# ntnu-arl/mimosa

Measured on AMD Instinct MI355X. Metric: ICP corr+residual Mpts/sec, 131k-pt scan vs 5M-pt map, 1/2/4/8 GPU, higher is better.
Workload: dtype f64; 1 GPU; configs[1]: OS0-128 131072-pt scan vs 4963194-pt local map (511380 voxels, 2x5 rooms), k=5 point-to-plane, ENWIDE params, cold linearize per step; parallelism=single GPU, exact_fallback_queries=0

## Files before the change

### mimosa_amd/csrc/icp_kernels.hip

```cpp
#include <hip/hip_runtime.h>

#include <cstdlib>

#include "icp_device.hpp"

#ifndef MH_PRUNE_TRIPS
#define MH_PRUNE_TRIPS (trip == 1 || trip == 2)
#endif
#ifndef MH_PIPE
#define MH_PIPE 4
#endif
#ifndef MH_XCD_PIECES
#define MH_XCD_PIECES 2
#endif
#ifndef MH_PIPE_SMALL
#define MH_PIPE_SMALL 4
#endif
#include "map_device.hpp"
#include "math3.hpp"
#include "wave_dpp.hpp"

namespace mh
{
namespace
// ... 93 lines not shown
#endif
#ifdef MH_TIMELINE
#define MH_STAMP4(ptr, i)                                                                                          \
  do {                                                                                                             \
    if ((ptr) && (threadIdx.x & 63) == 0 && (threadIdx.x >> 6) < static_cast<unsigned int>(NW))                    \
      (ptr)[(static_cast<size_t>(block_id) * NW + (threadIdx.x >> 6)) * 16 + (i)] = __builtin_amdgcn_s_memtime();  \
  } while (0)
#else
#define MH_STAMP4(ptr, i) do { } while (0)
#endif
#define MH_STAMP_C2(ptr, i) MH_STAMP(ptr, i)

struct KeyConsts
{
  uint32_t ymask, ymagic, kmask, xmask, xmagic;
};

__device__ __forceinline__ void cmp_exch(uint32_t & a, uint32_t & b)
{
  const uint32_t lo = min(a, b);
  b = max(a, b);
  a = lo;
}

typedef float f32x2 __attribute__((ext_vector_type(2)));
__device__ __forceinline__ uint32_t med3_u32(uint32_t a, uint32_t b, uint32_t c)
{
  uint32_t r;
  asm("v_med3_u32 %0, %1, %2, %3" : "=v"(r) : "v"(a), "v"(b), "v"(c));
  return r;
}
__device__ __forceinline__ f32x2 coarse_dist2(const KeyConsts & kc, uint32_t wa, uint32_t wb, float ofx, float mfy, float ofz)
{
  const f32x2 xm = {__uint_as_float((wa & kc.xmask) | kc.xmagic), __uint_as_float((wb & kc.xmask) | kc.xmagic)};
  const f32x2 x = xm - 8388608.0f;
  const f32x2 y = {__uint_as_float((wa & kc.ymask) | kc.ymagic), __uint_as_float((wb & kc.ymask) | kc.ymagic)};
  const f32x2 z = {static_cast<float>(wa >> 20), static_cast<float>(wb >> 20)};
  const f32x2 dx = x + ofx, dy = y - mfy, dz = z + ofz;
  f32x2 d = dy * dy;
  d = __builtin_elementwise_fma(dx, dx, d);
  d = __builtin_elementwise_fma(dz, dz, d);
  return d;
}
template <int KK>
__device__ __forceinline__ void merge_quad(uint32_t (&ck)[KK], const KeyConsts & kc, const uint4 qw, float ofx, float mfy, float ofz,
                                           uint32_t pb, uint32_t vcnt)
{
  const f32x2 da = coarse_dist2(kc, qw.x, qw.y, ofx, mfy, ofz), db = coarse_dist2(kc, qw.z, qw.w, ofx, mfy, ofz);
  uint32_t k0 = (__float_as_uint(da.x) & kc.kmask) | pb;
  uint32_t k1 = (__float_as_uint(da.y) & kc.kmask) | (pb | 1u);
  uint32_t k2 = (__float_as_uint(db.x) & kc.kmask) | (pb | 2u);
  uint32_t k3 = (__float_as_uint(db.y) & kc.kmask) | (pb | 3u);
  k0 = vcnt > 0u ? k0 : 0xFFFFFFFFu;
  k1 = vcnt > 1u ? k1 : 0xFFFFFFFFu;
  k2 = vcnt > 2u ? k2 : 0xFFFFFFFFu;
  k3 = vcnt > 3u ? k3 : 0xFFFFFFFFu;
  if constexpr (KK == 8) {
    cmp_exch(k0, k1); cmp_exch(k2, k3); cmp_exch(k0, k2); cmp_exch(k1, k3); cmp_exch(k1, k2);
    const uint32_t q[4] = {k3, k2, k1, k0};
#pragma unroll
    for (int i = 0; i < 4; ++i) {
      const uint32_t hi = med3_u32(ck[i], ck[4 + i], q[i]);
      ck[i] = min(ck[i], q[i]);
      ck[4 + i] = hi;
    }
    cmp_exch(ck[0], ck[2]); cmp_exch(ck[1], ck[3]); cmp_exch(ck[4], ck[6]); cmp_exch(ck[5], ck[7]);
    cmp_exch(ck[0], ck[1]); cmp_exch(ck[2], ck[3]); cmp_exch(ck[4], ck[5]); cmp_exch(ck[6], ck[7]);
  } else {
    const uint32_t kq[4] = {k0, k1, k2, k3};
#pragma unroll
    for (int c = 0; c < 4; ++c) {
      uint32_t t = kq[c];
#pragma unroll
      for (int i = 0; i < KK - 1; ++i) {
        const uint32_t lo = min(ck[i], t);
        t = max(ck[i], t);
        ck[i] = lo;
      }
      ck[KK - 1] = min(ck[KK - 1], t);
    }
  }
}

struct ScanStage
{
  uint4 quad;
  float4 ofs;
  uint32_t pb;
  uint32_t vcnt;
};
template <int NOFF>
struct ScanCursor
{
  uint32_t rem;
  int o_cur = 0;
  uint32_t qd = 8u, nq_cur = 0u;
  uint64_t qc0, qc1;

  __device__ __forceinline__ ScanStage advance(const uint32_t * list, int lds_stride, const float4 * lut4, const uint4 * qbuckets)
  {
    const bool sw = (qd >= nq_cur) && rem != 0u;
    o_cur = sw ? __builtin_ctz(rem) : o_cur;
    rem = sw ? (rem & (rem - 1u)) : rem;
    qd = sw ? 0u : qd;
    if constexpr (NOFF <= 21)
      nq_cur = static_cast<uint32_t>(qc0 >> (3 * o_cur)) & 7u;
    else
      nq_cur = static_cast<uint32_t>((o_cur < 21 ? qc0 : qc1) >> (3 * (o_cur < 21 ? o_cur : o_cur - 21))) & 7u;
    const uint32_t e = list[o_cur * lds_stride];
    ScanStage st;
    st.ofs = lut4[o_cur];
    uint32_t qidx = (e >> 5) * (kBucketStride / 4) + min(qd, static_cast<uint32_t>(kBucketStride / 4 - 1));
    st.quad = qbuckets[qidx];
    const uint32_t q4 = qd << 2;
    st.vcnt = static_cast<uint32_t>(min(max(static_cast<int>(e & 31u) - static_cast<int>(q4), 0), 4));
    st.pb = (static_cast<uint32_t>(o_cur) << 5) | q4;
    ++qd;
    return st;
  }
};

template <int K, int KK, int NOFF>
__device__ __forceinline__ uint32_t prune_keep_mask(const uint32_t (&ck)[KK], const float (&boxd)[NOFF], int k, float err_g,
                                                    uint32_t kth_given = 0xFFFFFFFFu)
{
  uint32_t kth = kth_given;
#pragma unroll
  for (int i = 0; i < K; ++i)
    if (i == k - 1) kth = min(kth, ck[i]);
  const float kv = __uint_as_float(kth & ~0x3FFu) * (1.0f + 2.5e-4f);
  const float r_up = sqrtf(kv) * (1.0f + 2e-6f) + err_g;
  const float b_up = kth != 0xFFFFFFFFu ? r_up * r_up : 3.0e38f;
  uint32_t keep = ~0u;
#pragma unroll
  for (int b = 1; b < NOFF; ++b) keep &= boxd[b] > b_up ? ~(1u << b) : ~0u;
  return keep;
}

template <int NOFF>
__device__ __forceinline__ void box_dists(const float qg0, const float qg1, const float qg2, float (&boxd)[NOFF])
{
  constexpr int row = NOFF == 7 ? 1 : (NOFF == 19 ? 2 : 3);
  constexpr float kQ = static_cast<float>(1 << kQuantBits);
  const float marg = 1e-2f;
  const float gxm = fmaxf(qg0 - marg, 0.f), gxp = fmaxf(kQ - qg0 - marg, 0.f);
  const float gym = fmaxf(qg1 - marg, 0.f), gyp = fmaxf(kQ - qg1 - marg, 0.f);
  const float gzm = fmaxf(qg2 - marg, 0.f), gzp = fmaxf(kQ - qg2 - marg, 0.f);
  const float g2x[3] = {gxm * gxm, 0.f, gxp * gxp}, g2y[3] = {gym * gym, 0.f, gyp * gyp}, g2z[3] = {gzm * gzm, 0.f, gzp * gzp};
#pragma unroll
  for (int b = 0; b < NOFF; ++b) {
    const uint32_t ent = kScan.ent[row][b];
    boxd[b] = g2x[ent & 3u] + g2y[(ent >> 2) & 3u] + g2z[(ent >> 4) & 3u];
  }
}

template <int KK, int NOFF, int PIPE>
__device__ __forceinline__ uint32_t scan_trip(ScanCursor<NOFF> & cur, ScanStage (&stage)[PIPE], uint32_t (&ck)[KK], const KeyConsts & kc,
                                              const uint32_t * list, int lds_stride, const float4 * lut4, const uint4 * qbuckets,
                                              const float cx0, const float cy1, const float cz2, uint32_t & n_scanned)
{
  uint32_t live_quads = 0u;
#pragma unroll
  for (int u = 0; u < PIPE; ++u) {
    const ScanStage st = stage[u];
    stage[u] = cur.advance(list, lds_stride, lut4, qbuckets);
    n_scanned += st.vcnt;
    live_quads += st.vcnt ? 1u : 0u;
    merge_quad<KK>(ck, kc, st.quad, st.ofs.x + cx0, cy1 - st.ofs.y, st.ofs.z + cz2, st.pb, st.vcnt);
  }
  return live_quads;
}

template <int CTRL>
__device__ __forceinline__ uint32_t quad_pull(uint32_t v)
{
  return static_cast<uint32_t>(__builtin_amdgcn_update_dpp(0, static_cast<int>(v), CTRL, 0xF, 0xF, false));
}
template <int CTRL>
__device__ __forceinline__ void quad_merge8(uint32_t (&ck)[8])
{
  uint32_t o[8];
#pragma unroll
  for (int i = 0; i < 8; ++i) o[i] = quad_pull<CTRL>(ck[7 - i]);
#pragma unroll
  for (int i = 0; i < 8; ++i) ck[i] = min(ck[i], o[i]);
  cmp_exch(ck[0], ck[4]); cmp_exch(ck[1], ck[5]); cmp_exch(ck[2], ck[6]); cmp_exch(ck[3], ck[7]);
  cmp_exch(ck[0], ck[2]); cmp_exch(ck[1], ck[3]); cmp_exch(ck[4], ck[6]); cmp_exch(ck[5], ck[7]);
  cmp_exch(ck[0], ck[1]); cmp_exch(ck[2], ck[3]); cmp_exch(ck[4], ck[5]); cmp_exch(ck[6], ck[7]);
}
template <int QL>
__device__ __forceinline__ void group_merge8(uint32_t (&ck)[8])
{
  if constexpr (QL >= 2) quad_merge8<0xB1>(ck);
  if constexpr (QL >= 4) quad_merge8<0x4E>(ck);
}
template <int QL>
__device__ __forceinline__ uint32_t group_min(uint32_t v)
{
  if constexpr (QL >= 2) v = min(v, quad_pull<0xB1>(v));
  if constexpr (QL >= 4) v = min(v, quad_pull<0x4E>(v));
  return v;
}
template <int QL>
__device__ __forceinline__ uint32_t group_or(uint32_t v)
{
  if constexpr (QL >= 2) v |= quad_pull<0xB1>(v);
  if constexpr (QL >= 4) v |= quad_pull<0x4E>(v);
  return v;
}
__device__ __forceinline__ uint32_t prefix_parity(uint32_t x)
{
  uint32_t y = x;
  y ^= y << 1;
  y ^= y << 2;
  y ^= y << 4;
  y ^= y << 8;
  y ^= y << 16;
  return y;
}
template <int QL>
__device__ __forceinline__ uint32_t deal_bits(uint32_t x, uint32_t sub)
{
  if constexpr (QL == 1) return x;
  const uint32_t odd = x & prefix_parity(x);
  uint32_t m = (sub & 1u) ? (x & ~odd) : odd;
  if constexpr (QL == 4) {
    const uint32_t odd2 = m & prefix_parity(m);
    m = (sub & 2u) ? (m & ~odd2) : odd2;
  }
  return m;
}

template <int KK>
struct KnnPoints
{
  float4 pt[KK];
  uint32_t member;
};
constexpr int knn_survivors(int K) { return K + 3 + (K > 5 ? 1 : 0); }
template <int K, int NOFF, bool FAST = false, int PIPE = MH_PIPE, int QL = 1>
__device__ __forceinline__ uint32_t knn_query(const MapView & map, const double q0, const double q1, const double q2,
                                              int k, uint32_t * list, int lds_stride, const uint32_t * scan_lut,
                                              uint32_t (&bi)[K], double & dk, bool & fell_back, uint32_t & n_scanned,
                                              unsigned long long * dbg = nullptr, KnnPoints<knn_survivors(K)> * fast = nullptr)
{
  (void)dbg;
  (void)fast;
  static_assert(QL == 1 || (FAST && knn_survivors(K) == 8), "several lanes per query: the k = 5 fast path's top-8 only");
  [[maybe_unused]] const uint32_t sub = QL > 1 ? (threadIdx.x & static_cast<uint32_t>(QL - 1)) : 0u;
  fell_back = false;
  constexpr int KK = knn_survivors(K);
  constexpr int row = NOFF == 7 ? 1 : (NOFF == 19 ? 2 : 3);
  const double u0 = q0 * map.inv_leaf, u1 = q1 * map.inv_leaf, u2 = q2 * map.inv_leaf;
  const int cx = fast_floor(u0), cy = fast_floor(u1), cz = fast_floor(u2);
  constexpr int m = kBlockDim - 1;
  const int bx = cx >> kBlockLog2, by = cy >> kBlockLog2, bz = cz >> kBlockLog2;
  int blk_id;
  {
    const uint64_t key = pack_coord_key(bx, by, bz);
    const int klo = static_cast<int>(static_cast<uint32_t>(key)), khi = static_cast<int>(static_cast<uint32_t>(key >> 32));
    uint32_t h = block_hash(bx, by, bz) & map.mask;
    int4 e = map.table[h];
    while (e.y != -1 && !(e.x == klo && e.y == khi)) {
      h = (h + 1) & map.mask;
      e = map.table[h];
    }
    constexpr int kB = 1 << (kVoxCoordBits - 1 - kBlockLog2);
    const bool in_range = ((static_cast<uint32_t>(bx + kB) | static_cast<uint32_t>(by + kB) | static_cast<uint32_t>(bz + kB)) >> (kVoxCoordBits - kBlockLog2)) == 0u;
    blk_id = (e.y != -1 && in_range) ? e.z : -1;
  }
  MH_STAMP(dbg, 8);
  uint32_t col[9][3];
  {
    const uint32_t * tab = map.cells + static_cast<size_t>(blk_id < 0 ? 0 : blk_id) * kCellsPerBlock +
                           halo_index(cx & m, cy & m, cz & m);
#pragma unroll
    for (int c = 0; c < 9; ++c) {
      const uint32_t * p = tab + ((c / 3 - 1) * kHaloDim + (c % 3 - 1)) * kHaloDim - 1;
      col[c][0] = p[0];
      col[c][1] = p[1];
      col[c][2] = p[2];
    }
  }
  uint32_t cell[NOFF];
#pragma unroll
  for (int b = 0; b < NOFF; ++b) {
    const uint32_t ent = kScan.ent[row][b];
    const int ox = static_cast<int>(ent & 3u), oy = static_cast<int>((ent >> 2) & 3u), oz = static_cast<int>((ent >> 4) & 3u);
    cell[b] = (blk_id >= 0 && static_cast<int>(ent >> 6) < map.n_off) ? col[ox * 3 + oy][oz] : kEmptyCell;
  }
#ifdef MH_TIMELINE
  asm volatile("s_waitcnt vmcnt(0)" ::: "memory");
#endif
  MH_STAMP(dbg, 9);
  uint32_t amask = 0u, total_ref = 0u;
  uint64_t qc0 = 0, qc1 = 0;
#pragma unroll
  for (int o = 0; o < NOFF; ++o) {
    static_assert(kEmptyCell == 0u, "an empty cell reads as (voxel 0, count 0): a mapped index and no candidates, without a select");
    list[o * lds_stride] = cell[o];
    const uint32_t c = cell[o] & 31u;
    amask |= (c ? 1u : 0u) << o;
    total_ref += c;
    const uint64_t nq = (c + 3u) >> 2;
    if (o < 21)
      qc0 |= nq << (3 * o);
    else
      qc1 |= nq << (3 * (o - 21));
  }
  MH_STAMP(dbg, 1);

  constexpr float kErrG = 0.9f;
  constexpr double kQ_d = static_cast<double>(1 << kQuantBits);
  const float qg0 = static_cast<float>((u0 - static_cast<double>(cx)) * kQ_d);
  const float qg1 = static_cast<float>((u1 - static_cast<double>(cy)) * kQ_d);
  const float qg2 = static_cast<float>((u2 - static_cast<double>(cz)) * kQ_d);
  uint32_t ck[KK];
#pragma unroll
  for (int i = 0; i < KK; ++i) ck[i] = 0xFFFFFFFFu;
  KeyConsts kc{0xFFC00u, 0x46000000u, ~0x3FFu, 0x3FFu, 0x4B000000u};
  asm volatile("" : "+v"(kc.ymask), "+v"(kc.ymagic), "+v"(kc.kmask), "+v"(kc.xmask), "+v"(kc.xmagic));

  n_scanned = 0;
  if constexpr (QL == 1) {
    if (amask & 1u) {
      const uint32_t cc = cell[0] & 31u;
      const uint4 * b = map.qbuckets + static_cast<size_t>(cell[0] >> 5) * (kBucketStride / 4);
      n_scanned += cc;
      const float ofx = 0.5f - qg0, ofy = 0.5f - qg1, ofz = 0.5f - qg2;
      uint4 qw[kBucketStride / 4];
#pragma unroll
      for (int u = 0; u < kBucketStride / 4; ++u) qw[u] = b[static_cast<uint32_t>(4 * u) < cc ? u : 0];
#pragma unroll
      for (int u = 0; u < kBucketStride / 4; ++u) {
        if (static_cast<uint32_t>(4 * u) < cc) merge_quad<KK>(ck, kc, qw[u], ofx, 8192.0f - ofy, ofz, static_cast<uint32_t>(4 * u), min(cc - static_cast<uint32_t>(4 * u), 4u));
      }
    }
  } else {
    const uint32_t cc = cell[0] & 31u;
    const uint4 * b = map.qbuckets + static_cast<size_t>(cell[0] >> 5) * (kBucketStride / 4);
    const float ofx = 0.5f - qg0, ofy = 0.5f - qg1, ofz = 0.5f - qg2;
    constexpr int NJ = (kBucketStride / 4 + QL - 1) / QL;
    uint4 qw[NJ];
#pragma unroll
    for (int j = 0; j < NJ; ++j) qw[j] = b[min(static_cast<uint32_t>(j * QL) + sub, static_cast<uint32_t>(kBucketStride / 4 - 1))];
#pragma unroll
    for (int j = 0; j < NJ; ++j) {
      const uint32_t u4 = 4u * (static_cast<uint32_t>(j * QL) + sub);
      const uint32_t vc = static_cast<uint32_t>(min(max(static_cast<int>(cc) - static_cast<int>(u4), 0), 4));
      n_scanned += vc;
      merge_quad<KK>(ck, kc, qw[j], ofx, 8192.0f - ofy, ofz, min(u4, 28u), vc);
    }
    group_merge8<QL>(ck);
  }
  MH_STAMP(dbg, 10);
  float boxd[NOFF];
  box_dists<NOFF>(qg0, qg1, qg2, boxd);
  uint32_t rem = amask & ~1u;
  rem &= prune_keep_mask<K, KK, NOFF>(ck, boxd, k, kErrG);
  [[maybe_unused]] uint32_t kth_group = 0xFFFFFFFFu;
  if constexpr (QL > 1) {
#pragma unroll
    for (int i = 0; i < K; ++i)
      if (i == k - 1) kth_group = ck[i];
    rem = deal_bits<QL>(rem, sub);
    if (sub != 0u) {
#pragma unroll
      for (int i = 0; i < KK; ++i) ck[i] = 0xFFFFFFFFu;
    }
  }
  uint32_t alive = rem;

  MH_STAMP(dbg, 11);
  {
    constexpr int kPipe = PIPE;
    const float4 * lut4 = reinterpret_cast<const float4 *>(scan_lut);
    const float cx0 = 0.5f - qg0, cy1 = 8192.0f - 0.5f + qg1, cz2 = 0.5f - qg2;
    ScanCursor<NOFF> cur;
    cur.rem = rem;
    cur.qc0 = qc0;
    cur.qc1 = qc1;
    ScanStage stage[kPipe];
#pragma unroll
    for (int u = 0; u < kPipe; ++u) stage[u] = cur.advance(list, lds_stride, lut4, map.qbuckets);
    for (int trip = 0;; ++trip) {
      if (!__any(static_cast<int>(stage[0].vcnt))) break;
      if (MH_PRUNE_TRIPS) {
        if constexpr (QL > 1) {
          uint32_t mine = kth_group;
#pragma unroll
          for (int i = 0; i < K; ++i)
            if (i == k - 1) mine = min(mine, ck[i]);
          kth_group = group_min<QL>(mine);
        }
        const uint32_t keep = prune_keep_mask<K, KK, NOFF>(ck, boxd, k, kErrG, kth_group);
        cur.rem &= keep;
        alive &= keep;
      }
      scan_trip<KK, NOFF, kPipe>(cur, stage, ck, kc, list, lds_stride, lut4, map.qbuckets, cx0, cy1, cz2, n_scanned);
    }
    rem = cur.rem;
  }
  if constexpr (QL > 1) {
    group_merge8<QL>(ck);
    alive = group_or<QL>(alive & ~rem);
    rem = 0u;
  }
  const uint32_t lane = threadIdx.x & 63u;
  const uint64_t act = __ballot(1);
  const uint32_t nact = static_cast<uint32_t>(__popcll(act));
  const uint32_t rank = static_cast<uint32_t>(__popcll(act & ((1ull << lane) - 1ull)));
  const uint32_t scanned_mask = (amask & 1u) | (alive & ~rem);
  MH_STAMP(dbg, 2);

  double bd[K];
  uint32_t br[K];
#pragma unroll
  for (int i = 0; i < K; ++i) {
    bd[i] = kDblMax;
    bi[i] = 0xFFFFFFFFu;
    br[i] = 0xFFFFFFFFu;
  }
  {
    uint32_t sidx[KK], srank[KK];
    float4 sc[KK];
#pragma unroll
    for (int u = 0; u < KK; ++u) {
      const uint32_t p = ck[u] & 0x3FFu;
      const int b = min(static_cast<int>(p >> 5), NOFF - 1);
      const uint32_t e = list[b * lds_stride];
      sidx[u] = (e >> 5) * kBucketStride + (p & 31u);
      sc[u] = map.buckets[sidx[u]];
      srank[u] = (scan_lut[4 * b + 3] << 5) | (p & 31u);
    }
    if constexpr (FAST) {
      unsigned long long d[KK];
      uint32_t rk[KK];
#pragma unroll
      for (int u = 0; u < KK; ++u) {
        const double du = sq_dist3(static_cast<double>(sc[u].x) - q0, static_cast<double>(sc[u].y) - q1, static_cast<double>(sc[u].z) - q2);
        d[u] = static_cast<unsigned long long>(__double_as_longlong(ck[u] != 0xFFFFFFFFu ? du : kDblMax));
        rk[u] = 0u;
      }
#pragma unroll
      for (int u = 0; u < KK; ++u)
#pragma unroll
        for (int v = u + 1; v < KK; ++v) {
          const bool lt = d[u] < d[v];
          rk[v] += lt ? 1u : 0u;
          rk[u] += lt ? 0u : 1u;
        }
      unsigned long long dk_bits = static_cast<unsigned long long>(__double_as_longlong(kDblMax)), dn_bits = ~0ull;
#pragma unroll
      for (int u = 0; u < KK; ++u) {
        dk_bits = rk[u] == static_cast<uint32_t>(k - 1) ? d[u] : dk_bits;
        dn_bits = rk[u] == static_cast<uint32_t>(k) ? d[u] : dn_bits;
      }
      uint32_t member = 0u;
#pragma unroll
      for (int u = 0; u < KK; ++u) {
        const bool valid = ck[u] != 0xFFFFFFFFu;
        member |= (valid && rk[u] < static_cast<uint32_t>(k)) ? (1u << u) : 0u;
        fast->pt[u] = sc[u];
      }
      if (__any(static_cast<int>(dk_bits == dn_bits && dk_bits != static_cast<unsigned long long>(__double_as_longlong(kDblMax))))) {
        uint32_t rt[KK];
#pragma unroll
        for (int u = 0; u < KK; ++u) rt[u] = 0u;
#pragma unroll
        for (int u = 0; u < KK; ++u)
#pragma unroll
          for (int v = u + 1; v < KK; ++v) {
            const bool lt = d[u] < d[v] || (d[u] == d[v] && srank[u] < srank[v]);
            rt[v] += lt ? 1u : 0u;
            rt[u] += lt ? 0u : 1u;
          }
        uint32_t mt = 0u;
#pragma unroll
        for (int u = 0; u < KK; ++u) mt |= (ck[u] != 0xFFFFFFFFu && rt[u] < static_cast<uint32_t>(k)) ? (1u << u) : 0u;
        member = mt;
// ... 235 lines not shown
  __syncthreads();
  return *s_last;
}

template <int EW, int TPB, bool PLAIN = false, int BATCH = 16>
__device__ __forceinline__ void fold_rows(const double * partials, int n_blocks, int n_ent, double * s_seg,
                                          double * s_out)
{
  constexpr int NSEG = (TPB < 256 ? TPB : 256) / EW;
  const int ent = threadIdx.x % EW, seg = threadIdx.x / EW;
  if (seg < NSEG && ent < n_ent) {
    constexpr int kBatch = BATCH;
    double acc = 0.0;
    for (int b0 = seg; b0 < n_blocks; b0 += kBatch * NSEG) {
      double v[kBatch];
#pragma unroll
      for (int u = 0; u < kBatch; ++u) {
        const int b = b0 + u * NSEG;
        const double * src = partials + static_cast<size_t>(b < n_blocks ? b : seg) * kPartialStride + ent;
        v[u] = PLAIN ? *src : load_partial(src);
      }
#pragma unroll
      for (int u = 0; u < kBatch; ++u) acc += (b0 + u * NSEG < n_blocks) ? v[u] : 0.0;
    }
    s_seg[seg * EW + ent] = acc;
  } else if (seg < NSEG) {
    s_seg[seg * EW + ent] = 0.0;
  }
  __syncthreads();
  if (static_cast<int>(threadIdx.x) < n_ent) {
    double s = 0.0;
    for (int g = 0; g < NSEG; ++g) s += s_seg[g * EW + threadIdx.x];
    s_out[threadIdx.x] = s;
  }
  __syncthreads();
}

}

template <typename A>
__device__ __forceinline__ void loc_directions(const A & a, const double nx, const double ny, const double nz, const double px,
                                               const double py, const double pz, double (&jr)[3], double (&jt)[3])
{
  const double ns0 = a.R[0] * nx + (a.R[3] * ny + a.R[6] * nz);
  const double ns1 = a.R[1] * nx + (a.R[4] * ny + a.R[7] * nz);
  const double ns2 = a.R[2] * nx + (a.R[5] * ny + a.R[8] * nz);
  double r0 = ns1 * pz - ns2 * py, r1 = ns2 * px - ns0 * pz, r2 = ns0 * py - ns1 * px;
  const double nr2 = r0 * r0 + (r1 * r1 + r2 * r2);
  if (nr2 > 0.0) {
    const double inv = mh_rsqrt(nr2);
    r0 *= inv;
    r1 *= inv;
    r2 *= inv;
  }
  jr[0] = r0;
  jr[1] = r1;
  jr[2] = r2;
  jt[0] = -ns0;
  jt[1] = -ns1;
  jt[2] = -ns2;
}

template <int K, bool BINARY, int NOFF, int TPB, bool SHARD, int QL = 1>
__device__ __forceinline__ void icp_linearize_body(const IcpArgs & a, const int block_id, const int n_blocks)
{
  static_assert(QL == 1 || (!SHARD && K == 5), "several lanes per query: plain k = 5 factors only");
  constexpr int PPW = TPB / QL;
  [[maybe_unused]] const bool lead = QL == 1 || (threadIdx.x & static_cast<unsigned int>(QL - 1)) == 0u;
  constexpr int NV = BINARY ? 13 : 7;
  constexpr int NENT = NV * (NV + 1) / 2;
  constexpr int EW = BINARY ? 96 : 32;
  constexpr int ROWW = NV;
  constexpr int kListWords = NOFF * PPW;
  constexpr int kFoldWords = (TPB / EW) * EW * 2 + EW * 2;
  constexpr int kArenaWords = kListWords > kFoldWords ? kListWords : kFoldWords;
  __shared__ __attribute__((aligned(16))) uint32_t s_arena[kArenaWords];
  __shared__ double s_tile[TPB * ROWW];
  __shared__ double s_wsum[(TPB / 64) * (NENT <= 32 ? 2 : 1) * NENT];
  __shared__ unsigned int s_cnt[4];
  __shared__ uint32_t s_scan[kScanLutWords];
  __shared__ bool s_last;

  uint32_t * s_list = s_arena + threadIdx.x / QL;
  double * s_aux = reinterpret_cast<double *>(s_arena);

#if !defined(MH_NO_INTERLEAVE)
  const int qi = [&] {
    if constexpr (QL > 1) return xcd_chunk(block_id, n_blocks) * PPW + static_cast<int>(threadIdx.x) / QL;
    constexpr int WPB = TPB / 64;
    const int cpx = n_blocks >> 3, x = block_id & 7, j = block_id >> 3, wv = static_cast<int>(threadIdx.x >> 6);
#if MH_XCD_PIECES > 1
    constexpr int P = MH_XCD_PIECES;
    static_assert(WPB % P == 0, "pieces must divide the waves of a workgroup");
    const int S = cpx * (WPB / P), p = wv / (WPB / P), o = (wv % (WPB / P)) * cpx + j;
    return ((p * 8 + ((p & 1) ? 7 - x : x)) * S + o) * 64 + static_cast<int>(threadIdx.x & 63u);
#else
    return ((x * cpx * WPB) + wv * cpx + j) * 64 + static_cast<int>(threadIdx.x & 63u);
#endif
  }();
#else
  const int qi = xcd_chunk(block_id, n_blocks) * PPW + static_cast<int>(threadIdx.x) / QL;
#endif
  const int k = (K == 5) ? 5 : a.k;
  const int n_pts = SHARD ? static_cast<int>(*a.n_dev) : a.n;
  float4 sp = make_float4(0.f, 0.f, 0.f, 0.f);
  if (qi < n_pts) sp = a.src[qi];
  if (threadIdx.x < 4) s_cnt[threadIdx.x] = 0u;
  fill_scan_lut<NOFF>(s_scan);
  __syncthreads();

  double row[NV];
  [[maybe_unused]] double rec_jr[3] = {0.0, 0.0, 0.0}, rec_jt[3] = {0.0, 0.0, 0.0};
  [[maybe_unused]] int rec_st = -1;
  uint32_t cnt_pack = 0u;
  bool did_knn = false, did_fall = false;
#ifdef MH_TIMELINE
  for (int rep = 0; rep < a.reps; ++rep) {
  if (rep > 0) {
    __syncthreads();
    if (threadIdx.x < 4) s_cnt[threadIdx.x] = 0u;
    __syncthreads();
  }
#endif
  MH_STAMP(a.dbg, 0);
#pragma unroll
  for (int j = 0; j < NV; ++j) row[j] = 0.0;

  if (qi < n_pts) {
    const double px = sp.x, py = sp.y, pz = sp.z;
    const double q0 = (a.R[0] * px + (a.R[1] * py + a.R[2] * pz)) + a.t[0];
    const double q1 = (a.R[3] * px + (a.R[4] * py + a.R[5] * pz)) + a.t[1];
    const double q2 = (a.R[6] * px + (a.R[7] * py + a.R[8] * pz)) + a.t[2];

    double qd0 = 0.0, qd1 = 0.0, qd2 = 0.0;
    int st = MH_UNPROCESSED;
    if (!a.cold) {
      qd0 = a.q_da[3 * qi + 0];
      qd1 = a.q_da[3 * qi + 1];
      qd2 = a.q_da[3 * qi + 2];
      st = a.status[qi];
    }
    bool gone = SHARD && (st & kShardSkip) != 0;
    if constexpr (SHARD) {
      if (a.cold) {
        const int raw = a.status[qi];
        gone = (raw & kShardSkip) != 0;
        if (gone && raw != -1) {
          a.status[qi] = kShardSkip;
          a.q_da[3 * qi + 0] = a.q_da[3 * qi + 1] = a.q_da[3 * qi + 2] = 0.0;
          a.mean[3 * qi + 0] = a.mean[3 * qi + 1] = a.mean[3 * qi + 2] = 0.0;
          a.normal[3 * qi + 0] = a.normal[3 * qi + 1] = a.normal[3 * qi + 2] = 0.0;
        }
      }
    }
    const double ddx = q0 - qd0, ddy = q1 - qd1, ddz = q2 - qd2;
    const bool update = !gone && (ddx * ddx + (ddy * ddy + ddz * ddz)) > a.da_thresh * a.da_thresh;

    double mean[3] = {0, 0, 0}, nrm[3] = {0, 0, 0};
    bool go = false;
    if (update) {
      st = MH_UNPROCESSED;
      if (lead) {
        a.q_da[3 * qi + 0] = q0;
        a.q_da[3 * qi + 1] = q1;
        a.q_da[3 * qi + 2] = q2;
      }
      uint32_t bi[K];
      double dk;
      bool fell_back;
      uint32_t n_scanned;
      constexpr bool kFast = K == 5;
      constexpr int KS = knn_survivors(K);
      [[maybe_unused]] KnnPoints<KS> sel;
      constexpr int kPipeK3 = TPB <= 256 ? MH_PIPE_SMALL : MH_PIPE;
      const uint32_t n_cand = knn_query<K, NOFF, kFast, kPipeK3, QL>(a.map, q0, q1, q2, k, s_list, PPW, s_scan, bi, dk, fell_back, n_scanned, a.dbg,
                                                                            kFast ? &sel : nullptr);
      cnt_pack = (lead ? n_cand : 0u) | (n_scanned << 16);
      did_knn = lead;
      did_fall = fell_back;
      if (!(dk < kDblMax)) {
        st = MH_INSUFFICIENT_CORRES_POINTS;
      } else if (dk > a.max_d2) {
        st = MH_CORRES_MAX_DIST;
      } else {
        constexpr int NX = kFast ? KS : K;
        double X[NX][3];
        [[maybe_unused]] double dm[NX];
        double sx = 0, sy = 0, sz = 0;
        if constexpr (kFast) {
#pragma unroll
          for (int j = 0; j < NX; ++j) {
            const bool m = (sel.member >> j) & 1u;
            X[j][0] = static_cast<double>(m ? sel.pt[j].x : 0.0f);
            X[j][1] = static_cast<double>(m ? sel.pt[j].y : 0.0f);
            X[j][2] = static_cast<double>(m ? sel.pt[j].z : 0.0f);
            dm[j] = __hiloint2double(m ? 0x3FF00000 : 0, 0);
            sx += X[j][0];
            sy += X[j][1];
            sz += X[j][2];
          }
        } else {
#pragma unroll
          for (int j = 0; j < K; ++j) {
            X[j][0] = X[j][1] = X[j][2] = 0.0;
            if (j < k) {
              const float4 c = a.map.buckets[bi[j]];
              X[j][0] = c.x;
              X[j][1] = c.y;
              X[j][2] = c.z;
              sx += X[j][0];
              sy += X[j][1];
              sz += X[j][2];
            }
          }
        }
        MH_STAMP_C2(a.dbg, 13);
        const double kd = static_cast<double>(k);
        const double ikd = 1.0 / kd;
        mean[0] = sx * ikd;
        mean[1] = sy * ikd;
        mean[2] = sz * ikd;
        double c00 = 0, c01 = 0, c02 = 0, c11 = 0, c12 = 0, c22 = 0;
#pragma unroll
        for (int j = 0; j < NX; ++j) {
          if constexpr (kFast) {
            X[j][0] = fma(-dm[j], mean[0], X[j][0]);
            X[j][1] = fma(-dm[j], mean[1], X[j][1]);
            X[j][2] = fma(-dm[j], mean[2], X[j][2]);
          } else {
            const bool m = j < k;
            X[j][0] = m ? X[j][0] - mean[0] : 0.0;
            X[j][1] = m ? X[j][1] - mean[1] : 0.0;
            X[j][2] = m ? X[j][2] - mean[2] : 0.0;
          }
          c00 += X[j][0] * X[j][0];
          c01 += X[j][0] * X[j][1];
          c02 += X[j][0] * X[j][2];
          c11 += X[j][1] * X[j][1];
          c12 += X[j][1] * X[j][2];
          c22 += X[j][2] * X[j][2];
        }
        const double ikm1 = 1.0 / (kd - 1.0);
        if (lead) {
          a.mean[3 * qi + 0] = mean[0];
          a.mean[3 * qi + 1] = mean[1];
          a.mean[3 * qi + 2] = mean[2];
        }
        double w[3], v0[3];
        MH_STAMP_C2(a.dbg, 14);
        plane_eigen(c00 * ikm1, c01 * ikm1, c02 * ikm1, c11 * ikm1, c12 * ikm1, c22 * ikm1, w, v0);
        MH_STAMP_C2(a.dbg, 15);
        if (!(w[0] == w[0]) || !(w[2] == w[2])) {
          st = MH_EIGEN_SOLVER_FAIL;
        } else if (w[0] < 1e-6) {
          st = MH_MIN_EIGEN_VALUE_LOW;
        } else if (w[2] > 3.0 * w[1]) {
          st = MH_LINE;
        } else {
          nrm[0] = v0[0];
// ... 423 lines not shown
      ll_store(ll_rows + threadIdx.x, s, a.seq);
    } else if (threadIdx.x < 8) {
      const int h0 = threadIdx.x == 6 ? 0 : 5, hn = threadIdx.x == 6 ? 5 : 4;
      unsigned long long pk = 0ull;
      for (int h = 0; h < hn; ++h) {
        unsigned int c = 0u;
        for (int w2 = 0; w2 < NW; ++w2) c += static_cast<unsigned int>(s_w[w2][6 + h0 + h]);
        pk |= static_cast<unsigned long long>(c) << (12 * h);
      }
      ll_rows[threadIdx.x] = make_uint4(static_cast<unsigned int>(pk), a.seq, static_cast<unsigned int>(pk >> 32), a.seq);
    }
    if (block_id == 0) {
      const int n_ent = a.nv * (a.nv + 1) / 2 + 4;
      if (threadIdx.x >= 64 && static_cast<int>(threadIdx.x) < 64 + n_ent) ll_store(a.ll + (threadIdx.x - 64), s_h[threadIdx.x - 64], a.seq);
      if (threadIdx.x >= 192 && threadIdx.x < 192 + 18) ll_store(a.ll + kLlSums + (threadIdx.x - 192), s_E[threadIdx.x - 192], a.seq);
    }
    (void)n_blocks;
    (void)s_last;
#ifdef MH_TIMELINE
    asm volatile("s_waitcnt vmcnt(0)" ::: "memory");
#endif
    MH_STAMP4(a.dbg, 9);
    return;
  } else {
  if (threadIdx.x < 15) {
    double s = 0.0;
    for (int w2 = 0; w2 < NW; ++w2) s += s_w[w2][threadIdx.x];
    store_partial(&a.partials[static_cast<size_t>(block_id) * kPartialStride + threadIdx.x], s);
  }
  if (!arrive_is_last(a.ticket, static_cast<unsigned int>(n_blocks), &s_last)) return;
  double * s_sum = s_seg + (TPB / 32) * 32;
  fold_rows<32, TPB>(a.partials, n_blocks, 15, s_seg, s_sum);
  if (threadIdx.x < 6) a.result->loc_comp[threadIdx.x] = s_sum[threadIdx.x];
  if (threadIdx.x >= 6 && threadIdx.x < 15)
    a.result->status_hist[threadIdx.x - 6] = static_cast<unsigned int>(s_sum[threadIdx.x]);
  if (a.shard_out && threadIdx.x < 16) a.shard_out[threadIdx.x] = threadIdx.x < 15 ? s_sum[threadIdx.x] : 0.0;
  if (threadIdx.x >= 32 && threadIdx.x < 50) {
    const int q = threadIdx.x - 32;
    double * dst = q < 9 ? &a.result->eig_rot[q] : &a.result->eig_trans[q - 9];
    *dst = s_E[q];
    if (a.host_result) *(q < 9 ? &a.host_result->eig_rot[q] : &a.host_result->eig_trans[q - 9]) = s_E[q];
  }
  if (a.host_result) {
    if (threadIdx.x < 6) a.host_result->loc_comp[threadIdx.x] = s_sum[threadIdx.x];
    if (threadIdx.x >= 6 && threadIdx.x < 15)
      a.host_result->status_hist[threadIdx.x - 6] = static_cast<unsigned int>(s_sum[threadIdx.x]);
  }
  }
}

template <int TPB, bool SHARD>
__global__ __launch_bounds__(loc_threads(TPB, SHARD)) void icp_localizability_kernel(const LocArgs a)
{
  icp_localizability_body<loc_tpb(TPB, SHARD), SHARD, loc_ch(TPB, SHARD), !SHARD>(a, static_cast<int>(blockIdx.x), static_cast<int>(gridDim.x));
}
template <int TPB>
__global__ __launch_bounds__(loc_tpb(TPB, false)) void icp_localizability_batch_kernel(const LocArgs * args, const int * start, int n_factors)
{
  const int b = static_cast<int>(blockIdx.x);
  const int f = batch_factor_of(start, n_factors, b);
  const int s0 = __builtin_amdgcn_readfirstlane(start[f]), s1 = __builtin_amdgcn_readfirstlane(start[f + 1]);
  const LocArgs a = load_uniform(args + f);
  icp_localizability_body<loc_tpb(TPB, false), false, loc_ch(TPB, false)>(a, b - s0, s1 - s0);
}

template <int TPB, bool SHARD>
__global__ __launch_bounds__(loc_tpb(TPB, SHARD)) void icp_localizability_batch_inline_kernel(const BatchInline<LocArgs> blk)
{
  (void)blk;
  const auto * p = (const BatchInline<LocArgs> *)__builtin_amdgcn_kernarg_segment_ptr();
  const int b = static_cast<int>(blockIdx.x);
  const int f = batch_factor_of(p->start, p->n, b);
  const int s0 = __builtin_amdgcn_readfirstlane(p->start[f]), s1 = __builtin_amdgcn_readfirstlane(p->start[f + 1]);
  const LocArgs a = load_uniform(p->a + f);
  icp_localizability_body<loc_tpb(TPB, SHARD), SHARD, loc_ch(TPB, SHARD)>(a, b - s0, s1 - s0);
}

__global__ __launch_bounds__(kThreads) void map_knn_kernel(const MapView map, const double * q, int n, int k,
                                                           double * pts, double * sq, int32_t * found)
{
  constexpr int K = 8;
  __shared__ uint32_t s_list[kMaxOff * kThreads];
  __shared__ uint32_t s_scan[kScanLutWords];
  if (map.n_off <= 7)
    fill_scan_lut<7>(s_scan);
  else if (map.n_off == 19)
    fill_scan_lut<19>(s_scan);
  else
    fill_scan_lut<27>(s_scan);
  __syncthreads();
  const int i = blockIdx.x * kThreads + threadIdx.x;
  if (i >= n) return;
  const double q0 = q[3 * i], q1 = q[3 * i + 1], q2 = q[3 * i + 2];
  uint32_t bi[K];
  double dk;
  bool fell_back;
  uint32_t n_scanned;
  if (map.n_off <= 7)
    knn_query<K, 7>(map, q0, q1, q2, k, s_list + threadIdx.x, kThreads, s_scan, bi, dk, fell_back, n_scanned);
  else if (map.n_off == 19)
    knn_query<K, 19>(map, q0, q1, q2, k, s_list + threadIdx.x, kThreads, s_scan, bi, dk, fell_back, n_scanned);
  else
    knn_query<K, 27>(map, q0, q1, q2, k, s_list + threadIdx.x, kThreads, s_scan, bi, dk, fell_back, n_scanned);
  int f = 0;
#pragma unroll
  for (int j = 0; j < K; ++j) {
    if (j < k) {
      const size_t o = static_cast<size_t>(i) * k + j;
      if (bi[j] != 0xFFFFFFFFu) {
        ++f;
        const float4 c = map.buckets[bi[j]];
        pts[o * 3 + 0] = c.x;
        pts[o * 3 + 1] = c.y;
        pts[o * 3 + 2] = c.z;
        sq[o] = sq_dist3(static_cast<double>(c.x) - q0, static_cast<double>(c.y) - q1, static_cast<double>(c.z) - q2);
      } else {
        pts[o * 3 + 0] = pts[o * 3 + 1] = pts[o * 3 + 2] = 0.0;
        sq[o] = kDblMax;
      }
    }
  }
  found[i] = f;
}

#ifndef MH_QL2_MAX
#define MH_QL2_MAX 32768
#endif
#ifndef MH_QL4_MAX
#define MH_QL4_MAX 0
#endif
static int env_or(const char * name, int dflt)
{
  const char * e = std::getenv(name);
  return (e && *e) ? std::atoi(e) : dflt;
}
int linearize_class(int n, int k, bool shard, long long total)
{
  static const int ql2_max = env_or("MH_QL2_MAX", MH_QL2_MAX), ql4_max = env_or("MH_QL4_MAX", MH_QL4_MAX);
  const long long tot = total > 0 ? total : n;
  if (!shard && k == 5) {
    if (tot <= ql4_max) return 64;
    if (tot <= ql2_max) return 128;
  }
  if (!shard && tot > 65536) return kThreads;
  return n <= 65536 ? 256 : kThreads;
}
int class_grid(int n, int ppw) { return (((n + ppw - 1) / ppw) + 7) & ~7; }
int linearize_grid_max(int n) { return class_grid(n, 64); }
static int loc_chunks(bool shard, int ppw) { return shard ? 1 : (kLocChunks * 256) / ppw; }
int class_loc_grid(int n, int ppw, bool shard)
{
  const int c = loc_chunks(shard, ppw);
  return (class_grid(n, ppw) + c - 1) / c;
}

template <int K, bool BINARY, int NOFF, bool SHARD>
static void launch_linearize_k(const IcpArgs & a, int ppw, hipStream_t stream)
{
  const dim3 grid(class_grid(a.n, ppw));
  if (ppw == 512) {
    hipLaunchKernelGGL((icp_linearize_kernel<K, BINARY, NOFF, kThreads, SHARD>), grid, dim3(kThreads), 0, stream, a);
    return;
  }
  if constexpr (K == 5 && !SHARD) {
    if (ppw == 128) {
      hipLaunchKernelGGL((icp_linearize_kernel<K, BINARY, NOFF, 256, SHARD, 2>), grid, dim3(256), 0, stream, a);
      return;
    }
    if (ppw == 64) {
      hipLaunchKernelGGL((icp_linearize_kernel<K, BINARY, NOFF, 256, SHARD, 4>), grid, dim3(256), 0, stream, a);
      return;
    }
  }
  hipLaunchKernelGGL((icp_linearize_kernel<K, BINARY, NOFF, 256, SHARD>), grid, dim3(256), 0, stream, a);
}
template <int NOFF>
static void launch_linearize_n(const IcpArgs & a, bool binary, hipStream_t stream)
{
  const bool shard = a.n_dev != nullptr;
  const int ppw = linearize_class(a.n, a.k, shard);
#define MH_K3_GO(KK, BIN)                                       \
  do {                                                          \
    if (shard)                                                  \
      launch_linearize_k<KK, BIN, NOFF, true>(a, ppw, stream);  \
    else                                                        \
      launch_linearize_k<KK, BIN, NOFF, false>(a, ppw, stream); \
// ... 197 lines not shown
```

Measured before the change: 3186 Mpts/s.

## Hand over straggler lanes' remaining voxel scans to idle wave lanes via LDS

Once the prune trips are done and only a few lanes in a wave still have quads to scan, those owner lanes publish their remaining scan items into a per-wave LDS slot area. All active lanes pick up chunks, merge them into local top-K lists, and write the partial results back, which each owner merges into its own list. This targets tail divergence, where most lanes idle while a few stragglers keep scanning. It adds wave-level LDS syncs, reuses the row tile memory as scratch, and adds code size and register pressure.

```diff
diff --git a/mimosa_amd/csrc/icp_kernels.hip b/mimosa_amd/csrc/icp_kernels.hip
--- a/mimosa_amd/csrc/icp_kernels.hip
+++ b/mimosa_amd/csrc/icp_kernels.hip
@@ -199,6 +199,15 @@
   }
 }
 
+__device__ __forceinline__ void merge8_reversed(uint32_t (&ck)[8], const uint32_t (&o)[8])
+{
+#pragma unroll
+  for (int i = 0; i < 8; ++i) ck[i] = min(ck[i], o[i]);
+  cmp_exch(ck[0], ck[4]); cmp_exch(ck[1], ck[5]); cmp_exch(ck[2], ck[6]); cmp_exch(ck[3], ck[7]);
+  cmp_exch(ck[0], ck[2]); cmp_exch(ck[1], ck[3]); cmp_exch(ck[4], ck[6]); cmp_exch(ck[5], ck[7]);
+  cmp_exch(ck[0], ck[1]); cmp_exch(ck[2], ck[3]); cmp_exch(ck[4], ck[5]); cmp_exch(ck[6], ck[7]);
+}
+
 struct ScanStage
 {
   uint4 quad;
@@ -235,6 +244,20 @@
     ++qd;
     return st;
   }
+  __device__ __forceinline__ bool more() const { return qd < nq_cur || rem != 0u; }
+  __device__ __forceinline__ uint32_t next()
+  {
+    if (qd >= nq_cur) {
+      o_cur = __builtin_ctz(rem);
+      rem &= rem - 1u;
+      qd = 0u;
+      if constexpr (NOFF <= 21)
+        nq_cur = static_cast<uint32_t>(qc0 >> (3 * o_cur)) & 7u;
+      else
+        nq_cur = static_cast<uint32_t>((o_cur < 21 ? qc0 : qc1) >> (3 * (o_cur < 21 ? o_cur : o_cur - 21))) & 7u;
+    }
+    return (static_cast<uint32_t>(o_cur) << 3) | qd++;
+  }
 };
 
 template <int K, int KK, int NOFF>
@@ -288,6 +311,134 @@
   return live_quads;
 }
 
+constexpr int kHandoverTrip = 3;
+constexpr bool prune_frozen_from(int t0)
+{
+  for (int trip = t0; trip < 64; ++trip)
+    if (MH_PRUNE_TRIPS) return false;
+  return true;
+}
+static_assert(prune_frozen_from(kHandoverTrip), "the hand-over needs the set of voxels to scan to be final");
+constexpr int kHoQuads = 4;
+constexpr int kHoChunksLog2 = 2;
+constexpr int kHoSlotWords = 8;
+constexpr int ho_owners(int KK) { return KK == 8 ? 16 : 8; }
+constexpr int ho_words(int KK) { return 64 * (KK + 1) + kHoSlotWords * ho_owners(KK); }
+constexpr int kHoWords = ho_words(12);
+static_assert(ho_words(8) <= kHoWords, "");
+
+__device__ __forceinline__ void wave_lds_sync()
+{
+  __builtin_amdgcn_fence(__ATOMIC_RELEASE, "wavefront");
+  __builtin_amdgcn_wave_barrier();
+  __builtin_amdgcn_fence(__ATOMIC_ACQUIRE, "wavefront");
+}
+template <int KK>
+__device__ __forceinline__ void merge_sorted(uint32_t (&ck)[KK], const uint32_t * o)
+{
+  if constexpr (KK == 8) {
+    uint32_t r[8];
+#pragma unroll
+    for (int i = 0; i < 8; ++i) r[i] = o[7 - i];
+    merge8_reversed(ck, r);
+  } else {
+#pragma unroll
+    for (int c = 0; c < KK; ++c) {
+      uint32_t t = o[c];
+#pragma unroll
+      for (int i = 0; i < KK - 1; ++i) {
+        const uint32_t lo = min(ck[i], t);
+        t = max(ck[i], t);
+        ck[i] = lo;
+      }
+      ck[KK - 1] = min(ck[KK - 1], t);
+    }
+  }
+}
+template <int KK, int NOFF, int PIPE>
+__device__ __forceinline__ void scan_handover(ScanCursor<NOFF> & cur, ScanStage (&stage)[PIPE], uint32_t (&ck)[KK], const KeyConsts & kc,
+                                              const uint32_t * list, int lds_stride, const float4 * lut4, const uint4 * qbuckets,
+                                              const float cx0, const float cy1, const float cz2, uint32_t & n_scanned, uint32_t * ho,
+                                              const uint64_t live)
+{
+  constexpr int RW = KK + 1;
+  uint32_t * const slots = ho + 64 * RW;
+  const uint32_t lane = threadIdx.x & 63u;
+  const uint64_t act = __ballot(1), below = (1ull << lane) - 1ull;
+  const uint32_t nact = static_cast<uint32_t>(__popcll(act)), rank = static_cast<uint32_t>(__popcll(act & below));
+  const uint32_t nlive = static_cast<uint32_t>(__popcll(live)), orank = static_cast<uint32_t>(__popcll(live & below));
+  const bool owner = (live >> lane) & 1ull;
+  uint32_t lper = kHoChunksLog2;
+  while ((nlive << lper) > nact) --lper;
+  const uint32_t cap = static_cast<uint32_t>(kHoQuads) << lper;
+  for (bool first = true;; first = false) {
+    uint32_t n = 0u;
+    if (owner) {
+      uint32_t * slot = slots + kHoSlotWords * orank;
+      uint8_t * items = reinterpret_cast<uint8_t *>(slot + 4);
+      while (n < cap && cur.more()) items[n++] = static_cast<uint8_t>(cur.next());
+      slot[0] = lane | (n << 8);
+      slot[1] = __float_as_uint(cx0);
+      slot[2] = __float_as_uint(cy1);
+      slot[3] = __float_as_uint(cz2);
+    }
+    wave_lds_sync();
+    const uint32_t j = rank >> lper, c = rank & ((1u << lper) - 1u);
+    const uint32_t * os = slots + kHoSlotWords * (j < nlive ? j : 0u);
+    const uint32_t hdr = os[0];
+    const uint32_t nj = j < nlive ? hdr >> 8 : 0u;
+    const int dl = static_cast<int>(hdr & 63u) - static_cast<int>(lane);
+    const float hx = __uint_as_float(os[1]), hy = __uint_as_float(os[2]), hz = __uint_as_float(os[3]);
+    const uint32_t iw = os[4 + c];
+    ScanStage hs[kHoQuads];
+#pragma unroll
+    for (int u = 0; u < kHoQuads; ++u) {
+      const bool valid = static_cast<uint32_t>(kHoQuads) * c + static_cast<uint32_t>(u) < nj;
+      const uint32_t it = valid ? (iw >> (8 * u)) & 0xFFu : 0u;
+      const uint32_t o = it >> 3, q4 = (it & 7u) << 2;
+      const uint32_t e = list[static_cast<int>(o) * lds_stride + dl];
+      hs[u].ofs = lut4[o];
+      hs[u].quad = qbuckets[(e >> 5) * (kBucketStride / 4) + (it & 7u)];
+      hs[u].vcnt = valid ? static_cast<uint32_t>(min(max(static_cast<int>(e & 31u) - static_cast<int>(q4), 0), 4)) : 0u;
+      hs[u].pb = (o << 5) | q4;
+    }
+    if (first) {
+#pragma unroll
+      for (int u = 0; u < PIPE; ++u) {
+        n_scanned += stage[u].vcnt;
+        merge_quad<KK>(ck, kc, stage[u].quad, stage[u].ofs.x + cx0, cy1 - stage[u].ofs.y, stage[u].ofs.z + cz2, stage[u].pb, stage[u].vcnt);
+        stage[u].vcnt = 0u;
+      }
+    }
+    uint32_t hk[KK], hv = 0u;
+#pragma unroll
+    for (int i = 0; i < KK; ++i) hk[i] = 0xFFFFFFFFu;
+#pragma unroll
+    for (int u = 0; u < kHoQuads; ++u) {
+      hv += hs[u].vcnt;
+      merge_quad<KK>(hk, kc, hs[u].quad, hs[u].ofs.x + hx, hy - hs[u].ofs.y, hs[u].ofs.z + hz, hs[u].pb, hs[u].vcnt);
+    }
+    uint32_t * res = ho + RW * rank;
+#pragma unroll
+    for (int i = 0; i < KK; ++i) res[i] = hk[i];
+    res[KK] = hv;
+    wave_lds_sync();
+    if (owner) {
+      const uint32_t nch = (n + static_cast<uint32_t>(kHoQuads - 1)) / static_cast<uint32_t>(kHoQuads);
+      for (uint32_t h = 0; h < nch; ++h) {
+        const uint32_t * r = ho + RW * ((orank << lper) + h);
+        uint32_t o[KK];
+#pragma unroll
+        for (int i = 0; i < KK; ++i) o[i] = r[i];
+        n_scanned += r[KK];
+        merge_sorted<KK>(ck, o);
+      }
+    }
+    if (!__any(static_cast<int>(owner && cur.more()))) break;
+    wave_lds_sync();
+  }
+}
+
 template <int CTRL>
 __device__ __forceinline__ uint32_t quad_pull(uint32_t v)
 {
@@ -299,11 +450,7 @@
   uint32_t o[8];
 #pragma unroll
   for (int i = 0; i < 8; ++i) o[i] = quad_pull<CTRL>(ck[7 - i]);
-#pragma unroll
-  for (int i = 0; i < 8; ++i) ck[i] = min(ck[i], o[i]);
-  cmp_exch(ck[0], ck[4]); cmp_exch(ck[1], ck[5]); cmp_exch(ck[2], ck[6]); cmp_exch(ck[3], ck[7]);
-  cmp_exch(ck[0], ck[2]); cmp_exch(ck[1], ck[3]); cmp_exch(ck[4], ck[6]); cmp_exch(ck[5], ck[7]);
-  cmp_exch(ck[0], ck[1]); cmp_exch(ck[2], ck[3]); cmp_exch(ck[4], ck[5]); cmp_exch(ck[6], ck[7]);
+  merge8_reversed(ck, o);
 }
 template <int QL>
 __device__ __forceinline__ void group_merge8(uint32_t (&ck)[8])
@@ -359,10 +506,12 @@
 __device__ __forceinline__ uint32_t knn_query(const MapView & map, const double q0, const double q1, const double q2,
                                               int k, uint32_t * list, int lds_stride, const uint32_t * scan_lut,
                                               uint32_t (&bi)[K], double & dk, bool & fell_back, uint32_t & n_scanned,
-                                              unsigned long long * dbg = nullptr, KnnPoints<knn_survivors(K)> * fast = nullptr)
+                                              unsigned long long * dbg = nullptr, KnnPoints<knn_survivors(K)> * fast = nullptr,
+                                              uint32_t * ho = nullptr)
 {
   (void)dbg;
   (void)fast;
+  (void)ho;
   static_assert(QL == 1 || (FAST && knn_survivors(K) == 8), "several lanes per query: the k = 5 fast path's top-8 only");
   [[maybe_unused]] const uint32_t sub = QL > 1 ? (threadIdx.x & static_cast<uint32_t>(QL - 1)) : 0u;
   fell_back = false;
@@ -513,6 +662,15 @@
         const uint32_t keep = prune_keep_mask<K, KK, NOFF>(ck, boxd, k, kErrG, kth_group);
         cur.rem &= keep;
         alive &= keep;
+      }
+      if constexpr (QL == 1) {
+        if (trip >= kHandoverTrip) {
+          const uint64_t live = __ballot(stage[0].vcnt != 0u);
+          if (__popcll(live) <= ho_owners(KK)) {
+            scan_handover<KK, NOFF, kPipe>(cur, stage, ck, kc, list, lds_stride, lut4, map.qbuckets, cx0, cy1, cz2, n_scanned, ho, live);
+            break;
+          }
+        }
       }
       scan_trip<KK, NOFF, kPipe>(cur, stage, ck, kc, list, lds_stride, lut4, map.qbuckets, cx0, cy1, cz2, n_scanned);
     }
@@ -914,6 +1072,8 @@
   __shared__ bool s_last;
 
   uint32_t * s_list = s_arena + threadIdx.x / QL;
+  static_assert(sizeof(double) * 64 * ROWW >= sizeof(uint32_t) * kHoWords, "a wave's row tile holds the hand-over area");
+  uint32_t * s_ho = reinterpret_cast<uint32_t *>(s_tile + static_cast<size_t>(threadIdx.x >> 6) * 64 * ROWW);
   double * s_aux = reinterpret_cast<double *>(s_arena);
 
 #if !defined(MH_NO_INTERLEAVE)
@@ -1006,7 +1166,7 @@
       [[maybe_unused]] KnnPoints<KS> sel;
       constexpr int kPipeK3 = TPB <= 256 ? MH_PIPE_SMALL : MH_PIPE;
       const uint32_t n_cand = knn_query<K, NOFF, kFast, kPipeK3, QL>(a.map, q0, q1, q2, k, s_list, PPW, s_scan, bi, dk, fell_back, n_scanned, a.dbg,
-                                                                            kFast ? &sel : nullptr);
+                                                                            kFast ? &sel : nullptr, s_ho);
       cnt_pack = (lead ? n_cand : 0u) | (n_scanned << 16);
       did_knn = lead;
       did_fall = fell_back;
@@ -1596,6 +1756,7 @@
   constexpr int K = 8;
   __shared__ uint32_t s_list[kMaxOff * kThreads];
   __shared__ uint32_t s_scan[kScanLutWords];
+  __shared__ uint32_t s_ho[(kThreads / 64) * kHoWords];
   if (map.n_off <= 7)
     fill_scan_lut<7>(s_scan);
   else if (map.n_off == 19)
@@ -1611,11 +1772,14 @@
   bool fell_back;
   uint32_t n_scanned;
   if (map.n_off <= 7)
-    knn_query<K, 7>(map, q0, q1, q2, k, s_list + threadIdx.x, kThreads, s_scan, bi, dk, fell_back, n_scanned);
+    knn_query<K, 7>(map, q0, q1, q2, k, s_list + threadIdx.x, kThreads, s_scan, bi, dk, fell_back, n_scanned, nullptr, nullptr,
+                    s_ho + (threadIdx.x >> 6) * kHoWords);
   else if (map.n_off == 19)
-    knn_query<K, 19>(map, q0, q1, q2, k, s_list + threadIdx.x, kThreads, s_scan, bi, dk, fell_back, n_scanned);
+    knn_query<K, 19>(map, q0, q1, q2, k, s_list + threadIdx.x, kThreads, s_scan, bi, dk, fell_back, n_scanned, nullptr, nullptr,
+                    s_ho + (threadIdx.x >> 6) * kHoWords);
   else
-    knn_query<K, 27>(map, q0, q1, q2, k, s_list + threadIdx.x, kThreads, s_scan, bi, dk, fell_back, n_scanned);
+    knn_query<K, 27>(map, q0, q1, q2, k, s_list + threadIdx.x, kThreads, s_scan, bi, dk, fell_back, n_scanned, nullptr, nullptr,
+                    s_ho + (threadIdx.x >> 6) * kHoWords);
   int f = 0;
 #pragma unroll
   for (int j = 0; j < K; ++j) {
```

Result: no change. 3157 Mpts/s (-0.9%).
